# secondlaw-ai/skyrim

Hardware: AMD Instinct MI355X
Metric: 6-h forecast steps/sec on 721x1440 state, 1/2/4/8 MI355X; per-channel max rel-err vs ref (higher is better)
Workload: dtype f16; 1 GPU; Pangu 6-h autoregressive rollout, 721x1440x69 state (13 levels x 5 vars + 4 surface), random-init weights (64 M params), state resident in HBM, 1 ensemble membe; parallelism=single GPU, members=1, finite=True, rounding=compensated, term_plan=0x66f

## Files before the change

### skyrim_amd/csrc/fused_block2.hip

```cpp
#include "blockrow.h"
#include "launchers.h"

namespace skp {

template <int C_, int FM_, bool ONE_>
struct Blk2Shape {
    static constexpr bool ONE = ONE_;
    static constexpr int C = C_, FM = FM_, NWAVES = 4, THREADS = 64 * NWAVES, RD = 2;
    static constexpr int KS = C / 32, CF = C / 16, HID = 4 * C, NCH = HID / 32, NPB = C / 32, BM = NWAVES * FM * 16;
    static constexpr int SLOT_KIB = KS * 2;
    static constexpr int SLOT = SLOT_KIB * 1024, NSLOT = 2;
    static constexpr int T_PB = 0, T_G1 = C, T_E1 = 2 * C, T_B1 = 3 * C, T_B2 = 3 * C + HID, T_G2 = T_B2 + C, T_E2 = T_G2 + C;
    static constexpr int TAB = T_E2 + C;
    static constexpr int SMEM = NSLOT * SLOT + TAB * 4;
    static_assert(SLOT_KIB % NWAVES == 0 && NPB % 2 == 0 && NCH >= 3, "DMA pieces per wave; even projection block count");
    static_assert(SMEM <= 80 * 1024, "two workgroups per CU");
};

template <class T, class S>
__global__ void __launch_bounds__(S::THREADS) __attribute__((amdgpu_waves_per_eu(2, 2)))
proj_mlp2_kernel(const Block2Args<T> a) {
    constexpr int C = S::C, FM = S::FM, KS = S::KS, CF = S::CF, NCH = S::NCH, NPB = S::NPB, NWAVES = S::NWAVES, RD = S::RD;
    typedef typename OpT<T>::v8 v8;
    extern __shared__ __attribute__((aligned(16))) char smem[];
    float* tab = reinterpret_cast<float*>(smem + S::NSLOT * S::SLOT);
    const int tid = threadIdx.x, lane = tid & 63, l15 = lane & 15, g = lane >> 4;
    const int wave = __builtin_amdgcn_readfirstlane(tid >> 6);
    const unsigned lds_base = (unsigned)(size_t)smem;
    const char* lrd = smem + lane * 16;

    auto dma1 = [&](const T* src, unsigned dst) {
        const T* s = src + lane * 8;
#pragma unroll
        for (int i = 0; i < S::SLOT_KIB / NWAVES; ++i) {
            const int q = wave + i * NWAVES;
            glds16(s + (q << 9), dst + (unsigned)(q << 10));
        }
    };
    dma1(a.projh, lds_base);

    for (int i = tid; i < C; i += S::THREADS) {
        tab[S::T_PB + i] = a.proj_b[i]; tab[S::T_G1 + i] = a.g1[i]; tab[S::T_E1 + i] = a.e1[i];
        tab[S::T_B2 + i] = a.b2[i]; tab[S::T_G2 + i] = a.g2[i]; tab[S::T_E2 + i] = a.e2[i];
    }
    for (int i = tid; i < S::HID; i += S::THREADS) tab[S::T_B1 + i] = a.b1[i];

    const long long rb0 = (long long)blockIdx.x * (S::BM / 16) + wave * FM;
    v8 xh[FM][KS], xl[FM][KS];
    bool live[FM];
#pragma unroll
    for (int t = 0; t < FM; ++t) {
        live[t] = (rb0 + t) * 16 < a.M;
        const int src = live[t] ? a.winv[(rb0 + t) * 16 + l15] : 0;
        const T* p = a.ao + blk_off(src, g * 8, C);
#pragma unroll
        for (int ks = 0; ks < KS; ++ks) {
            xh[t][ks] = *reinterpret_cast<const v8*>(p + (ks << 9));
            if constexpr (S::ONE) xl[t][ks] = v8{};
            else xl[t][ks] = *reinterpret_cast<const v8*>(p + (ks << 9) + a.ao_plane);
        }
    }
#pragma unroll
    for (int t = 0; t < FM; ++t) {
#pragma unroll
        for (int ks = 0; ks < KS; ++ks) {
            asm volatile("" : "+v"(xh[t][ks]));
            if constexpr (!S::ONE) asm volatile("" : "+v"(xl[t][ks]));
        }
    }

    f32x4 yacc[FM][CF];
#pragma unroll
    for (int t = 0; t < FM; ++t)
#pragma unroll
        for (int c = 0; c < CF; ++c) yacc[t][c] = f32x4{0.f, 0.f, 0.f, 0.f};

#pragma unroll
    for (int j = 0; j < NPB; ++j) {
        asm volatile("s_waitcnt vmcnt(0)" ::: "memory");
        __syncthreads();
        if (j + 1 < NPB) dma1(a.projh + ((long long)(j + 1) * S::SLOT_KIB << 9), lds_base + (unsigned)(((j + 1) & 1) * S::SLOT));
        else dma1(a.w1h, lds_base);
        sk_stream<KS, RD>(lrd + (j & 1) * S::SLOT, [&](int ks, const uint4& w0, const uint4& w1) {
            if constexpr (!S::ONE) {
#pragma unroll
                for (int t = 0; t < FM; ++t) yacc[t][2 * j] = OpT<T>::mfma(as_v8<T>(w0), xl[t][ks], yacc[t][2 * j]);
#pragma unroll
                for (int t = 0; t < FM; ++t) yacc[t][2 * j + 1] = OpT<T>::mfma(as_v8<T>(w1), xl[t][ks], yacc[t][2 * j + 1]);
            }
#pragma unroll
            for (int t = 0; t < FM; ++t) yacc[t][2 * j] = OpT<T>::mfma(as_v8<T>(w0), xh[t][ks], yacc[t][2 * j]);
#pragma unroll
            for (int t = 0; t < FM; ++t) yacc[t][2 * j + 1] = OpT<T>::mfma(as_v8<T>(w1), xh[t][ks], yacc[t][2 * j + 1]);
        });
    }

#pragma unroll
    for (int t = 0; t < FM; ++t) {
        const T* old = a.xs + ((live[t] ? rb0 + t : 0) * KS << 9) + l15 * 32 + g * 8;
        v8 oh[KS], ol[KS];
#pragma unroll
        for (int bp = 0; bp < KS; ++bp) {
            oh[bp] = *reinterpret_cast<const v8*>(old + (bp << 9));
            ol[bp] = *reinterpret_cast<const v8*>(old + (bp << 9) + a.xs_plane);
        }
        float s = 0.f;
#pragma unroll
        for (int bp = 0; bp < KS; ++bp) {
            const int n = 32 * bp + 8 * g;
            const float4 b0 = *reinterpret_cast<const float4*>(tab + S::T_PB + n), b1 = *reinterpret_cast<const float4*>(tab + S::T_PB + n + 4);
            add8(yacc[t][2 * bp], yacc[t][2 * bp + 1], b0, b1);
#pragma unroll
            for (int r = 0; r < 4; ++r) s += yacc[t][2 * bp][r] + yacc[t][2 * bp + 1][r];
        }
        s += __shfl_xor(s, 16);
        s += __shfl_xor(s, 32);
        const float mean = s * (1.0f / C);
        float q = 0.f;
#pragma unroll
        for (int c = 0; c < CF; ++c)
#pragma unroll
            for (int r = 0; r < 4; ++r) { const float d = yacc[t][c][r] - mean; q += d * d; }
        q += __shfl_xor(q, 16);
        q += __shfl_xor(q, 32);
        const float rstd = rsqrtf(q * (1.0f / C) + a.eps);
#pragma unroll
        for (int bp = 0; bp < KS; ++bp) {
            const int n = 32 * bp + 8 * g;
            const float4 g0 = *reinterpret_cast<const float4*>(tab + S::T_G1 + n), g1 = *reinterpret_cast<const float4*>(tab + S::T_G1 + n + 4);
            const float4 e0 = *reinterpret_cast<const float4*>(tab + S::T_E1 + n), e1 = *reinterpret_cast<const float4*>(tab + S::T_E1 + n + 4);
            const f32x4 &x = yacc[t][2 * bp], &z = yacc[t][2 * bp + 1];
            const float y[8] = {(x[0] - mean) * rstd * g0.x + e0.x, (x[1] - mean) * rstd * g0.y + e0.y, (x[2] - mean) * rstd * g0.z + e0.z, (x[3] - mean) * rstd * g0.w + e0.w,
                                (z[0] - mean) * rstd * g1.x + e1.x, (z[1] - mean) * rstd * g1.y + e1.y, (z[2] - mean) * rstd * g1.z + e1.z, (z[3] - mean) * rstd * g1.w + e1.w};
            float v[8];
#pragma unroll
            for (int i = 0; i < 8; ++i) v[i] = ((float)oh[bp][i] + (float)ol[bp][i]) + y[i];
            uint4 o[2];
            split8<T, 2>(v, o);
            xh[t][bp] = as_v8<T>(o[0]);
            xl[t][bp] = as_v8<T>(o[1]);
            asm volatile("" : "+v"(xh[t][bp]), "+v"(xl[t][bp]));
        }
#pragma unroll
        for (int c = 0; c < CF; ++c) yacc[t][c] = f32x4{0.f, 0.f, 0.f, 0.f};
    }

    f32x4 hacc[FM][2];
    uint4 hh[FM], hl[FM];
    for (int j = 0; j < NCH; ++j) {
        asm volatile("s_waitcnt vmcnt(0)" ::: "memory");
        __syncthreads();
        dma1(a.w2h + ((long long)j * S::SLOT_KIB << 9), lds_base + S::SLOT);
#pragma unroll
        for (int t = 0; t < FM; ++t) { hacc[t][0] = f32x4{0.f, 0.f, 0.f, 0.f}; hacc[t][1] = f32x4{0.f, 0.f, 0.f, 0.f}; }
        sk_stream<KS, RD>(lrd, [&](int ks, const uint4& w0, const uint4& w1) {
            if constexpr (!S::ONE) {
#pragma unroll
                for (int t = 0; t < FM; ++t) hacc[t][0] = OpT<T>::mfma(as_v8<T>(w0), xl[t][ks], hacc[t][0]);
#pragma unroll
                for (int t = 0; t < FM; ++t) hacc[t][1] = OpT<T>::mfma(as_v8<T>(w1), xl[t][ks], hacc[t][1]);
            }
#pragma unroll
            for (int t = 0; t < FM; ++t) hacc[t][0] = OpT<T>::mfma(as_v8<T>(w0), xh[t][ks], hacc[t][0]);
#pragma unroll
            for (int t = 0; t < FM; ++t) hacc[t][1] = OpT<T>::mfma(as_v8<T>(w1), xh[t][ks], hacc[t][1]);
        });
        {
            const float4 bb0 = *reinterpret_cast<const float4*>(tab + S::T_B1 + j * 32 + 4 * g), bb1 = *reinterpret_cast<const float4*>(tab + S::T_B1 + j * 32 + 16 + 4 * g);
#pragma unroll
            for (int t = 0; t < FM; ++t) {
                const f32x2 a0 = gelu_erf2(f32x2{hacc[t][0][0] + bb0.x, hacc[t][0][1] + bb0.y}), a1 = gelu_erf2(f32x2{hacc[t][0][2] + bb0.z, hacc[t][0][3] + bb0.w});
                const f32x2 a2 = gelu_erf2(f32x2{hacc[t][1][0] + bb1.x, hacc[t][1][1] + bb1.y}), a3 = gelu_erf2(f32x2{hacc[t][1][2] + bb1.z, hacc[t][1][3] + bb1.w});
                const float v[8] = {a0.x, a0.y, a1.x, a1.y, a2.x, a2.y, a3.x, a3.y};
                uint4 o[2];
                split8<T, 2>(v, o);
                hh[t] = o[0]; hl[t] = o[1];
            }
        }
        asm volatile("s_waitcnt vmcnt(0)" ::: "memory");
        __syncthreads();
        if (j + 1 < NCH) dma1(a.w1h + ((long long)(j + 1) * S::SLOT_KIB << 9), lds_base);
        sk_stream<CF / 2, RD>(lrd + S::SLOT, [&](int p, const uint4& w0, const uint4& w1) {
            if constexpr (!S::ONE) {
#pragma unroll
                for (int t = 0; t < FM; ++t) yacc[t][2 * p] = OpT<T>::mfma(as_v8<T>(w0), as_v8<T>(hl[t]), yacc[t][2 * p]);
#pragma unroll
                for (int t = 0; t < FM; ++t) yacc[t][2 * p + 1] = OpT<T>::mfma(as_v8<T>(w1), as_v8<T>(hl[t]), yacc[t][2 * p + 1]);
            }
#pragma unroll
            for (int t = 0; t < FM; ++t) yacc[t][2 * p] = OpT<T>::mfma(as_v8<T>(w0), as_v8<T>(hh[t]), yacc[t][2 * p]);
#pragma unroll
            for (int t = 0; t < FM; ++t) yacc[t][2 * p + 1] = OpT<T>::mfma(as_v8<T>(w1), as_v8<T>(hh[t]), yacc[t][2 * p + 1]);
        });
    }

#pragma unroll
    for (int t = 0; t < FM; ++t) {
        float s = 0.f;
#pragma unroll
        for (int bp = 0; bp < KS; ++bp) {
            const int n = 32 * bp + 8 * g;
            const float4 b0 = *reinterpret_cast<const float4*>(tab + S::T_B2 + n), b1 = *reinterpret_cast<const float4*>(tab + S::T_B2 + n + 4);
            add8(yacc[t][2 * bp], yacc[t][2 * bp + 1], b0, b1);
#pragma unroll
            for (int r = 0; r < 4; ++r) s += yacc[t][2 * bp][r] + yacc[t][2 * bp + 1][r];
        }
        s += __shfl_xor(s, 16);
        s += __shfl_xor(s, 32);
        const float mean = s * (1.0f / C);
        float q = 0.f;
#pragma unroll
        for (int c = 0; c < CF; ++c)
#pragma unroll
            for (int r = 0; r < 4; ++r) { const float d = yacc[t][c][r] - mean; q += d * d; }
        q += __shfl_xor(q, 16);
        q += __shfl_xor(q, 32);
        const float rstd = rsqrtf(q * (1.0f / C) + a.eps);
        if (!live[t]) continue;
        T* dst = a.xs + ((rb0 + t) * KS << 9) + l15 * 32 + g * 8;
#pragma unroll
        for (int bp = 0; bp < KS; ++bp) {
            const int n = 32 * bp + 8 * g;
            const float4 g0 = *reinterpret_cast<const float4*>(tab + S::T_G2 + n), g1 = *reinterpret_cast<const float4*>(tab + S::T_G2 + n + 4);
            const float4 e0 = *reinterpret_cast<const float4*>(tab + S::T_E2 + n), e1 = *reinterpret_cast<const float4*>(tab + S::T_E2 + n + 4);
            v8 mh = xh[t][bp], ml = xl[t][bp];
            asm volatile("" : "+v"(mh), "+v"(ml));
            float oh[8], ol[8];
#pragma unroll
            for (int i = 0; i < 8; ++i) { oh[i] = (float)mh[i]; ol[i] = (float)ml[i]; }
            const f32x4 &x = yacc[t][2 * bp], &z = yacc[t][2 * bp + 1];
            const float v[8] = {(oh[0] + ol[0]) + ((x[0] - mean) * rstd * g0.x + e0.x), (oh[1] + ol[1]) + ((x[1] - mean) * rstd * g0.y + e0.y),
                                (oh[2] + ol[2]) + ((x[2] - mean) * rstd * g0.z + e0.z), (oh[3] + ol[3]) + ((x[3] - mean) * rstd * g0.w + e0.w),
                                (oh[4] + ol[4]) + ((z[0] - mean) * rstd * g1.x + e1.x), (oh[5] + ol[5]) + ((z[1] - mean) * rstd * g1.y + e1.y),
                                (oh[6] + ol[6]) + ((z[2] - mean) * rstd * g1.z + e1.z), (oh[7] + ol[7]) + ((z[3] - mean) * rstd * g1.w + e1.w)};
            store8_planes<T, 2>(dst + (bp << 9), a.xs_plane, v);
        }
    }
}

template <class T, class S>
static hipError_t launch_blk2(const Block2Args<T>& a, hipStream_t s) {
    auto kern = proj_mlp2_kernel<T, S>;
    hipError_t e = hipFuncSetAttribute(reinterpret_cast<const void*>(kern), hipFuncAttributeMaxDynamicSharedMemorySize, S::SMEM);
    if (e != hipSuccess) return e;
    const unsigned grid = (unsigned)((a.M + S::BM - 1) / S::BM);
    if (grid == 0) return hipSuccess;
    hipLaunchKernelGGL(kern, dim3(grid), dim3(S::THREADS), S::SMEM, s, a);
    return hipGetLastError();
}

hipError_t op_proj_mlp2(const Geom& g, const BlockW<f16>& b, const int* winv, int res, f16* Xs, const Work<PrecF16x3>& wk, hipStream_t s, int one) {
    typedef f16 T;
    Block2Args<T> a{wk.ao, wk.ao_plane, g.ntok[res], Xs, wk.xs_plane[res], winv, b.projh, b.w1h, b.w2h,
                    b.proj_b, b.n1_g, b.n1_b, b.fc1_b, b.fc2_b, b.n2_g, b.n2_b, 1e-5f};
    if (a.M % 16 != 0) return hipErrorInvalidValue;
    if (res == 0) return one ? launch_blk2<T, Blk2Shape<192, 2, true>>(a, s) : launch_blk2<T, Blk2Shape<192, 2, false>>(a, s);
    return one ? launch_blk2<T, Blk2Shape<384, 1, true>>(a, s) : launch_blk2<T, Blk2Shape<384, 1, false>>(a, s);
}

}
```

Measured before the change: 70.78 steps/s.

## Restructure projection GEMM to stream K-steps and overlap residual loads

The projection loop now iterates over K-slices instead of output column blocks. Each step DMAs the weight slice for the next K step and waits only for the activation loads that step needs, using partial vmcnt waits. The residual (xs) loads are spread across the K loop so their latency hides behind MFMA work instead of stalling before the LayerNorm epilogue. This costs more live registers to hold the residual tiles for all rows and adds more complex wait-count bookkeeping.

```diff
diff --git a/skyrim_amd/csrc/fused_block2.hip b/skyrim_amd/csrc/fused_block2.hip
--- a/skyrim_amd/csrc/fused_block2.hip
+++ b/skyrim_amd/csrc/fused_block2.hip
@@ -7,20 +7,23 @@
 struct Blk2Shape {
     static constexpr bool ONE = ONE_;
     static constexpr int C = C_, FM = FM_, NWAVES = 4, THREADS = 64 * NWAVES, RD = 2;
-    static constexpr int KS = C / 32, CF = C / 16, HID = 4 * C, NCH = HID / 32, NPB = C / 32, BM = NWAVES * FM * 16;
+    static constexpr int KS = C / 32, CF = C / 16, HID = 4 * C, NCH = HID / 32, BM = NWAVES * FM * 16;
     static constexpr int SLOT_KIB = KS * 2;
     static constexpr int SLOT = SLOT_KIB * 1024, NSLOT = 2;
     static constexpr int T_PB = 0, T_G1 = C, T_E1 = 2 * C, T_B1 = 3 * C, T_B2 = 3 * C + HID, T_G2 = T_B2 + C, T_E2 = T_G2 + C;
     static constexpr int TAB = T_E2 + C;
     static constexpr int SMEM = NSLOT * SLOT + TAB * 4;
-    static_assert(SLOT_KIB % NWAVES == 0 && NPB % 2 == 0 && NCH >= 3, "DMA pieces per wave; even projection block count");
+    static_assert(SLOT_KIB % NWAVES == 0 && KS % 2 == 0 && NCH >= 3, "DMA pieces per wave; even projection step count");
     static_assert(SMEM <= 80 * 1024, "two workgroups per CU");
 };
+
+template <int N>
+__device__ __forceinline__ void vm_wait() { asm volatile("s_waitcnt vmcnt(%0)" ::"n"(N) : "memory"); }
 
 template <class T, class S>
 __global__ void __launch_bounds__(S::THREADS) __attribute__((amdgpu_waves_per_eu(2, 2)))
 proj_mlp2_kernel(const Block2Args<T> a) {
-    constexpr int C = S::C, FM = S::FM, KS = S::KS, CF = S::CF, NCH = S::NCH, NPB = S::NPB, NWAVES = S::NWAVES, RD = S::RD;
+    constexpr int C = S::C, FM = S::FM, KS = S::KS, CF = S::CF, NCH = S::NCH, NWAVES = S::NWAVES, RD = S::RD;
     typedef typename OpT<T>::v8 v8;
     extern __shared__ __attribute__((aligned(16))) char smem[];
     float* tab = reinterpret_cast<float*>(smem + S::NSLOT * S::SLOT);
@@ -37,7 +40,22 @@
             glds16(s + (q << 9), dst + (unsigned)(q << 10));
         }
     };
-    dma1(a.projh, lds_base);
+    auto dma1s = [&](const T* src, unsigned dst) {
+#pragma unroll
+        for (int i = 0; i < S::SLOT_KIB / NWAVES; ++i) {
+            const int q = wave + i * NWAVES;
+            glds16_s(src + (q << 9), (unsigned)lane * 16u, dst + (unsigned)(q << 10));
+        }
+    };
+    auto dma_ks = [&](int ks, unsigned dst) {
+#pragma unroll
+        for (int i = 0; i < CF / NWAVES; ++i) {
+            const int c = wave + i * NWAVES;
+            const int q = (c >> 1) * 2 * KS + 2 * ks + (c & 1);
+            glds16_s(a.projh + (q << 9), (unsigned)lane * 16u, dst + (unsigned)(c << 10));
+        }
+    };
+    dma_ks(0, lds_base);
 
     for (int i = tid; i < C; i += S::THREADS) {
         tab[S::T_PB + i] = a.proj_b[i]; tab[S::T_G1 + i] = a.g1[i]; tab[S::T_E1 + i] = a.e1[i];
@@ -48,62 +66,75 @@
     const long long rb0 = (long long)blockIdx.x * (S::BM / 16) + wave * FM;
     v8 xh[FM][KS], xl[FM][KS];
     bool live[FM];
+    const T *arow[FM], *old[FM];
 #pragma unroll
     for (int t = 0; t < FM; ++t) {
         live[t] = (rb0 + t) * 16 < a.M;
         const int src = live[t] ? a.winv[(rb0 + t) * 16 + l15] : 0;
-        const T* p = a.ao + blk_off(src, g * 8, C);
-#pragma unroll
-        for (int ks = 0; ks < KS; ++ks) {
-            xh[t][ks] = *reinterpret_cast<const v8*>(p + (ks << 9));
-            if constexpr (S::ONE) xl[t][ks] = v8{};
-            else xl[t][ks] = *reinterpret_cast<const v8*>(p + (ks << 9) + a.ao_plane);
-        }
-    }
-#pragma unroll
-    for (int t = 0; t < FM; ++t) {
-#pragma unroll
-        for (int ks = 0; ks < KS; ++ks) {
+        arow[t] = a.ao + blk_off(src, g * 8, C);
+        old[t] = a.xs + ((live[t] ? rb0 + t : 0) * KS << 9) + l15 * 32 + g * 8;
+    }
+#pragma unroll
+    for (int ks = 0; ks < KS; ++ks)
+#pragma unroll
+        for (int t = 0; t < FM; ++t) {
+            xh[t][ks] = *reinterpret_cast<const v8*>(arow[t] + (ks << 9));
+            if constexpr (!S::ONE) xl[t][ks] = *reinterpret_cast<const v8*>(arow[t] + (ks << 9) + a.ao_plane);
+        }
+
+    f32x4 yacc[FM][CF];
+#pragma unroll
+    for (int t = 0; t < FM; ++t)
+#pragma unroll
+        for (int c = 0; c < CF; ++c) yacc[t][c] = f32x4{0.f, 0.f, 0.f, 0.f};
+
+    constexpr int NPL = S::ONE ? 1 : 2;
+    constexpr int VM_0 = (KS - 1) * FM * NPL;
+    constexpr int VM_1 = S::ONE ? FM : 0;
+    constexpr int VM_N = FM * 2;
+    v8 oh[FM][KS], ol[FM][KS];
+#pragma unroll
+    for (int ks = 0; ks < KS; ++ks) {
+        if (ks == 0) vm_wait<VM_0>(); else if (ks == 1) vm_wait<VM_1>(); else vm_wait<VM_N>();
+#pragma unroll
+        for (int t = 0; t < FM; ++t) {
             asm volatile("" : "+v"(xh[t][ks]));
             if constexpr (!S::ONE) asm volatile("" : "+v"(xl[t][ks]));
         }
-    }
-
-    f32x4 yacc[FM][CF];
-#pragma unroll
-    for (int t = 0; t < FM; ++t)
-#pragma unroll
-        for (int c = 0; c < CF; ++c) yacc[t][c] = f32x4{0.f, 0.f, 0.f, 0.f};
-
-#pragma unroll
-    for (int j = 0; j < NPB; ++j) {
-        asm volatile("s_waitcnt vmcnt(0)" ::: "memory");
         __syncthreads();
-        if (j + 1 < NPB) dma1(a.projh + ((long long)(j + 1) * S::SLOT_KIB << 9), lds_base + (unsigned)(((j + 1) & 1) * S::SLOT));
-        else dma1(a.w1h, lds_base);
-        sk_stream<KS, RD>(lrd + (j & 1) * S::SLOT, [&](int ks, const uint4& w0, const uint4& w1) {
+        if (ks + 1 < KS) dma_ks(ks + 1, lds_base + (unsigned)(((ks + 1) & 1) * S::SLOT));
+        else dma1s(a.w1h, lds_base);
+        long long z = 0;
+        asm volatile("" : "+s"(z));
+#pragma unroll
+        for (int t = 0; t < FM; ++t) {
+            if constexpr (S::ONE) ol[t][ks] = *reinterpret_cast<const v8*>(old[t] + (z + (ks << 9) + a.xs_plane));
+            if (ks > 0) {
+                oh[t][ks - 1] = *reinterpret_cast<const v8*>(old[t] + (z + ((ks - 1) << 9)));
+                if constexpr (!S::ONE) ol[t][ks - 1] = *reinterpret_cast<const v8*>(old[t] + (z + ((ks - 1) << 9) + a.xs_plane));
+            }
+        }
+        sk_stream<CF / 2, RD>(lrd + (ks & 1) * S::SLOT, [&](int p, const uint4& w0, const uint4& w1) {
             if constexpr (!S::ONE) {
 #pragma unroll
-                for (int t = 0; t < FM; ++t) yacc[t][2 * j] = OpT<T>::mfma(as_v8<T>(w0), xl[t][ks], yacc[t][2 * j]);
-#pragma unroll
-                for (int t = 0; t < FM; ++t) yacc[t][2 * j + 1] = OpT<T>::mfma(as_v8<T>(w1), xl[t][ks], yacc[t][2 * j + 1]);
-            }
-#pragma unroll
-            for (int t = 0; t < FM; ++t) yacc[t][2 * j] = OpT<T>::mfma(as_v8<T>(w0), xh[t][ks], yacc[t][2 * j]);
-#pragma unroll
-            for (int t = 0; t < FM; ++t) yacc[t][2 * j + 1] = OpT<T>::mfma(as_v8<T>(w1), xh[t][ks], yacc[t][2 * j + 1]);
+                for (int t = 0; t < FM; ++t) yacc[t][2 * p] = OpT<T>::mfma(as_v8<T>(w0), xl[t][ks], yacc[t][2 * p]);
+#pragma unroll
+                for (int t = 0; t < FM; ++t) yacc[t][2 * p + 1] = OpT<T>::mfma(as_v8<T>(w1), xl[t][ks], yacc[t][2 * p + 1]);
+            }
+#pragma unroll
+            for (int t = 0; t < FM; ++t) yacc[t][2 * p] = OpT<T>::mfma(as_v8<T>(w0), xh[t][ks], yacc[t][2 * p]);
+#pragma unroll
+            for (int t = 0; t < FM; ++t) yacc[t][2 * p + 1] = OpT<T>::mfma(as_v8<T>(w1), xh[t][ks], yacc[t][2 * p + 1]);
         });
     }
-
-#pragma unroll
-    for (int t = 0; t < FM; ++t) {
-        const T* old = a.xs + ((live[t] ? rb0 + t : 0) * KS << 9) + l15 * 32 + g * 8;
-        v8 oh[KS], ol[KS];
-#pragma unroll
-        for (int bp = 0; bp < KS; ++bp) {
-            oh[bp] = *reinterpret_cast<const v8*>(old + (bp << 9));
-            ol[bp] = *reinterpret_cast<const v8*>(old + (bp << 9) + a.xs_plane);
-        }
+#pragma unroll
+    for (int t = 0; t < FM; ++t) {
+        oh[t][KS - 1] = *reinterpret_cast<const v8*>(old[t] + ((KS - 1) << 9));
+        if constexpr (!S::ONE) ol[t][KS - 1] = *reinterpret_cast<const v8*>(old[t] + ((KS - 1) << 9) + a.xs_plane);
+    }
+
+#pragma unroll
+    for (int t = 0; t < FM; ++t) {
         float s = 0.f;
 #pragma unroll
         for (int bp = 0; bp < KS; ++bp) {
@@ -123,9 +154,10 @@
             for (int r = 0; r < 4; ++r) { const float d = yacc[t][c][r] - mean; q += d * d; }
         q += __shfl_xor(q, 16);
         q += __shfl_xor(q, 32);
-        const float rstd = rsqrtf(q * (1.0f / C) + a.eps);
-#pragma unroll
-        for (int bp = 0; bp < KS; ++bp) {
+        float rstd = rsqrtf(q * (1.0f / C) + a.eps);
+#pragma unroll
+        for (int bp = 0; bp < KS; ++bp) {
+            asm volatile("" : "+v"(oh[t][bp]), "+v"(ol[t][bp]), "+v"(rstd));
             const int n = 32 * bp + 8 * g;
             const float4 g0 = *reinterpret_cast<const float4*>(tab + S::T_G1 + n), g1 = *reinterpret_cast<const float4*>(tab + S::T_G1 + n + 4);
             const float4 e0 = *reinterpret_cast<const float4*>(tab + S::T_E1 + n), e1 = *reinterpret_cast<const float4*>(tab + S::T_E1 + n + 4);
@@ -134,7 +166,7 @@
                                 (z[0] - mean) * rstd * g1.x + e1.x, (z[1] - mean) * rstd * g1.y + e1.y, (z[2] - mean) * rstd * g1.z + e1.z, (z[3] - mean) * rstd * g1.w + e1.w};
             float v[8];
 #pragma unroll
-            for (int i = 0; i < 8; ++i) v[i] = ((float)oh[bp][i] + (float)ol[bp][i]) + y[i];
+            for (int i = 0; i < 8; ++i) v[i] = ((float)oh[t][bp][i] + (float)ol[t][bp][i]) + y[i];
             uint4 o[2];
             split8<T, 2>(v, o);
             xh[t][bp] = as_v8<T>(o[0]);
```

Result: no change. 70.82 steps/s, median of 2 (+0.1%).
